# brdav/refign

Measured on AMD Instinct MI355X. Metric: image-pairs/s (align+seg fwd+bwd, 1080x1920), higher is better.
Workload: dtype bf16

## Files before the change

### refign_amd/csrc/attn.hip

```cpp
#include <cstdlib>

#include "common.h"
#include "mfma.h"

namespace rfn {

constexpr int kPackBlock = 4096;
constexpr float kLog2e = 1.4426950408889634f;

__global__ __launch_bounds__(256) void attn_pack_kernel(const uint16_t* __restrict__ src0, const uint16_t* __restrict__ src1,
                                                        long sb, long sr, int heads, int nrows, int nblk,
                                                        unsigned char* __restrict__ rpack0, unsigned char* __restrict__ tpack0,
                                                        unsigned char* __restrict__ rpack1, unsigned char* __restrict__ tpack1) {
  __shared__ unsigned tile[32][33];
  const uint16_t* src = blockIdx.z ? src1 : src0;
  unsigned char* rpack = blockIdx.z ? rpack1 : rpack0;
  unsigned char* tpack = blockIdx.z ? tpack1 : tpack0;
  const int blk = blockIdx.x, bh = blockIdx.y;
  const int b = bh / heads, hd = bh % heads;
  const int t = threadIdx.x, row = t >> 3, dc = t & 7;
  const int grow = blk * 32 + row;
  u32x4 v = {0u, 0u, 0u, 0u};
  if (grow < nrows) v = *(const u32x4*)(src + (long)b * sb + (long)grow * sr + hd * 64 + dc * 8);
  unsigned char* rb = rpack + ((long)bh * nblk + blk) * kPackBlock;
  if (rpack != nullptr) *(u32x4*)(rb + (dc * 32 + row) * 16) = v;
  if (tpack == nullptr) return;
  tile[row][dc * 4 + 0] = v[0];
  tile[row][dc * 4 + 1] = v[1];
  tile[row][dc * 4 + 2] = v[2];
  tile[row][dc * 4 + 3] = v[3];
  __syncthreads();
  const int rq = t >> 5, dp = t & 31;
  unsigned r0 = tile[4 * rq + 0][dp], r1 = tile[4 * rq + 1][dp], r2 = tile[4 * rq + 2][dp], r3 = tile[4 * rq + 3][dp];
  u32x4 o;
  o[0] = (r0 & 0xffffu) | (r1 << 16);
  o[1] = (r2 & 0xffffu) | (r3 << 16);
  o[2] = (r0 >> 16) | (r1 & 0xffff0000u);
  o[3] = (r2 >> 16) | (r3 & 0xffff0000u);
  unsigned char* tb = tpack + ((long)bh * nblk + blk) * kPackBlock;
  *(u32x4*)(tb + (rq * 64 + 2 * dp) * 8) = o;
}

template <int DT>
__device__ __forceinline__ void load_row_frags(const uint16_t* base, long row_stride, int row, int nrows, int g,
                                               typename Elem<DT>::vec8 (&f)[4]) {
  const bool ok = row < nrows;
  const uint16_t* p = base + (long)(ok ? row : 0) * row_stride + 8 * g;
#pragma unroll
  for (int ks = 0; ks < 4; ++ks) {
    u32x4 v = {0u, 0u, 0u, 0u};
    if (ok) v = *(const u32x4*)(p + 16 * ks);
    f[ks] = __builtin_bit_cast(typename Elem<DT>::vec8, v);
  }
}

template <int DT>
__device__ __forceinline__ void store_rows64(const f32x16 (&acc)[2], float mul, uint16_t* rowptr, bool ok, int g) {
#pragma unroll
  for (int db = 0; db < 2; ++db) {
    u32x2 pk[4];
#pragma unroll
    for (int k = 0; k < 4; ++k)
      pk[k] = pack4<DT>(acc[db][4 * k] * mul, acc[db][4 * k + 1] * mul, acc[db][4 * k + 2] * mul, acc[db][4 * k + 3] * mul);
#pragma unroll
    for (int p = 0; p < 2; ++p) {
      auto r0 = __builtin_amdgcn_permlane32_swap(pk[2 * p][0], pk[2 * p + 1][0], false, false);
      auto r1 = __builtin_amdgcn_permlane32_swap(pk[2 * p][1], pk[2 * p + 1][1], false, false);
      if (ok) {
        u32x4 o = {r0[0], r1[0], r0[1], r1[1]};
        *(u32x4*)(rowptr + db * 32 + 16 * p + 8 * g) = o;
      }
    }
  }
}

template <int DT>
__device__ __forceinline__ void to_operands(const float (&p)[16], typename Elem<DT>::vec8 (&b)[2]) {
#pragma unroll
  for (int m = 0; m < 2; ++m)
    b[m] = join8<DT>(pack4<DT>(p[8 * m], p[8 * m + 1], p[8 * m + 2], p[8 * m + 3]),
                     pack4<DT>(p[8 * m + 4], p[8 * m + 5], p[8 * m + 6], p[8 * m + 7]));
}

template <int DT>
__global__ __launch_bounds__(256) void attn_fwd_kernel(const uint16_t* __restrict__ Q, long qsb, long qsr,
                                                       const unsigned char* __restrict__ Kr,
                                                       const unsigned char* __restrict__ Vt, uint16_t* __restrict__ O,
                                                       long osb, long osr, float* __restrict__ lse2, int heads, int Nq,
                                                       int Nkv, int nblk, int nqpad, float scale, int pheads) {
  using E = Elem<DT>;
  using vec8 = typename E::vec8;
  constexpr int STAGE = 4 * kPackBlock;
  __shared__ __attribute__((aligned(16))) unsigned char smem[2 * STAGE];
  const int lane = threadIdx.x & 63, wave = threadIdx.x >> 6, g = lane >> 5, col = lane & 31;
  const int bh = blockIdx.y, b = bh / heads, hd = bh % heads;
  const int q = blockIdx.x * 128 + wave * 32 + col;
  const float c = scale * kLog2e;

  vec8 qf[4];
  load_row_frags<DT>(Q + (long)b * qsb + hd * 64, qsr, q, Nq, g, qf);
#pragma unroll
  for (int kk = 0; kk < 4; ++kk) pin_loaded(qf[kk]);

  const long pidx = (long)(b * pheads + hd) * nblk * kPackBlock;
  const unsigned char* kbase = Kr + pidx;
  const unsigned char* vbase = Vt + pidx;
  const int nst = nblk / 2;
  auto issue = [&](int st, int buf) {
    unsigned char* dst = smem + buf * STAGE;
#pragma unroll
    for (int u = 0; u < 2; ++u) {
      const int piece = wave * 2 + u;
      lds_dma16(kbase + (long)st * 2 * kPackBlock + piece * 1024 + lane * 16, dst + piece * 1024);
      lds_dma16(vbase + (long)st * 2 * kPackBlock + piece * 1024 + lane * 16, dst + 2 * kPackBlock + piece * 1024);
    }
  };

  f32x16 oacc[2];
#pragma unroll
  for (int r = 0; r < 16; ++r) oacc[0][r] = oacc[1][r] = 0.f;
  float mrun = -1e30f, lrun = 0.f;

  issue(0, 0);
  wait_dma_all();
  wg_barrier();
  for (int st = 0; st < nst; ++st) {
    const int buf = st & 1;
    if (st + 1 < nst) issue(st + 1, buf ^ 1);
    const unsigned char* ks = smem + buf * STAGE;
    const unsigned char* vs = ks + 2 * kPackBlock;
    const int key0 = st * 64;
    f32x16 sacc[2];
#pragma unroll
    for (int kb = 0; kb < 2; ++kb)
#pragma unroll
      for (int r = 0; r < 16; ++r) sacc[kb][r] = 0.f;
    {
      vec8 kfr[4];
      auto kfrag = [&](int idx) {
        return *(const vec8*)(ks + (idx >> 2) * kPackBlock + ((2 * (idx & 3) + g) * 32 + col) * 16);
      };
#pragma unroll
      for (int idx = 0; idx < 4; ++idx) kfr[idx] = kfrag(idx);
      __builtin_amdgcn_sched_barrier(0);
#pragma unroll
      for (int idx = 0; idx < 8; ++idx) {
        sacc[idx >> 2] = E::mma(kfr[idx & 3], qf[idx & 3], sacc[idx >> 2]);
        if (idx + 4 < 8) kfr[idx & 3] = kfrag(idx + 4);
        __builtin_amdgcn_sched_barrier(0);
      }
    }
    vec8 vfr[4];
    auto vfrag = [&](int idx) {
      const unsigned char* vq = vs + (idx >> 2) * kPackBlock + ((idx & 1) * 32 + col) * 8;
      const int m = (idx >> 1) & 1;
      return join8<DT>(*(const u32x2*)(vq + (4 * m + g) * 512), *(const u32x2*)(vq + (4 * m + 2 + g) * 512));
    };
#pragma unroll
    for (int idx = 0; idx < 4; ++idx) vfr[idx] = vfrag(idx);
    __builtin_amdgcn_sched_barrier(0);
    float p[2][16];
#pragma unroll
    for (int kb = 0; kb < 2; ++kb)
#pragma unroll
      for (int r = 0; r < 16; ++r) p[kb][r] = sacc[kb][r];
    if (key0 + 64 > Nkv) {
      asm volatile("; padded keys" ::: "memory");
#pragma unroll
      for (int kb = 0; kb < 2; ++kb)
#pragma unroll
        for (int r = 0; r < 16; ++r)
          if (key0 + kb * 32 + (r & 3) + 8 * (r >> 2) + 4 * g >= Nkv) p[kb][r] = -1e30f;
    }
    float mt = p[0][0];
#pragma unroll
    for (int kb = 0; kb < 2; ++kb)
#pragma unroll
      for (int r = 0; r < 16; ++r) mt = fmaxf(mt, p[kb][r]);
    mt = half_max(mt) * c;
    const float mnew = fmaxf(mrun, mt);
    if (__any(mnew > mrun)) {
      const float alpha = __builtin_amdgcn_exp2f(mrun - mnew);
      lrun *= alpha;
#pragma unroll
      for (int r = 0; r < 16; ++r) {
        oacc[0][r] *= alpha;
        oacc[1][r] *= alpha;
      }
      mrun = mnew;
    }
    float ps = 0.f;
#pragma unroll
    for (int kb = 0; kb < 2; ++kb)
#pragma unroll
      for (int r = 0; r < 16; ++r) {
        p[kb][r] = __builtin_amdgcn_exp2f(__builtin_fmaf(p[kb][r], c, -mrun));
        ps += p[kb][r];
      }
    lrun += ps;
    {
      vec8 pb[2][2];
      to_operands<DT>(p[0], pb[0]);
      to_operands<DT>(p[1], pb[1]);
#pragma unroll
      for (int idx = 0; idx < 8; ++idx) {
        const int kb = idx >> 2, m = (idx >> 1) & 1, db = idx & 1;
        oacc[db] = E::mma(vfr[idx & 3], pb[kb][m], oacc[db]);
        if (idx + 4 < 8) vfr[idx & 3] = vfrag(idx + 4);
        __builtin_amdgcn_sched_barrier(0);
      }
    }
    wait_dma_all();
    wg_barrier();
  }
  const float l = half_sum(lrun);
  const bool ok = q < Nq;
  store_rows64<DT>(oacc, 1.f / l, O + (long)b * osb + (long)(ok ? q : 0) * osr + hd * 64, ok, g);
  if (g == 0 && q < nqpad) lse2[(long)bh * nqpad + q] = ok ? mrun + log2f(l) : 0.f;
}


template <int DT>
__global__ __launch_bounds__(256) void attn_bwd_dq_kernel(const uint16_t* __restrict__ Q, long qsb, long qsr,
                                                          const uint16_t* __restrict__ dO, const uint16_t* __restrict__ O,
                                                          long osb, long osr, const unsigned char* __restrict__ Kr,
                                                          const unsigned char* __restrict__ Vr,
                                                          const unsigned char* __restrict__ Kt,
                                                          const float* __restrict__ lse2, float* __restrict__ delta,
                                                          uint16_t* __restrict__ dQ, long dsb, long dsr, int heads, int Nq,
                                                          int Nkv, int nblk, int nqpad, float scale, int pheads) {
  using E = Elem<DT>;
  using vec8 = typename E::vec8;
  constexpr int STAGE = 6 * kPackBlock;
  __shared__ __attribute__((aligned(16))) unsigned char smem[2 * STAGE];
  const int lane = threadIdx.x & 63, wave = threadIdx.x >> 6, g = lane >> 5, col = lane & 31;
  const int bh = blockIdx.y, b = bh / heads, hd = bh % heads;
  const int q = blockIdx.x * 128 + wave * 32 + col;
  const bool ok = q < Nq;
  const float c = scale * kLog2e;

  vec8 qf[4], gf[4];
  load_row_frags<DT>(Q + (long)b * qsb + hd * 64, qsr, q, Nq, g, qf);
  load_row_frags<DT>(dO + (long)b * osb + hd * 64, osr, q, Nq, g, gf);
  float dl = 0.f;
  {
    vec8 of[4];
    load_row_frags<DT>(O + (long)b * osb + hd * 64, osr, q, Nq, g, of);
#pragma unroll
    for (int kk = 0; kk < 4; ++kk)
#pragma unroll
      for (int e = 0; e < 8; ++e) dl += (float)gf[kk][e] * (float)of[kk][e];
    dl = half_sum(dl);
  }
  const float ls = (q < nqpad) ? lse2[(long)bh * nqpad + q] : 0.f;
  if (g == 0 && q < nqpad) delta[(long)bh * nqpad + q] = ok ? dl : 0.f;
#pragma unroll
  for (int kk = 0; kk < 4; ++kk) {
    pin_loaded(qf[kk]);
    pin_loaded(gf[kk]);
  }
  pin_loaded(ls);

  const long pbase = (long)(b * pheads + hd) * nblk * kPackBlock;
  const int nst = nblk / 2;
  auto issue = [&](int st, int buf) {
    unsigned char* dst = smem + buf * STAGE;
#pragma unroll
    for (int u = 0; u < 2; ++u) {
      const int piece = wave * 2 + u;
      const long off = pbase + (long)st * 2 * kPackBlock + piece * 1024 + lane * 16;
      lds_dma16(Kr + off, dst + piece * 1024);
      lds_dma16(Vr + off, dst + 2 * kPackBlock + piece * 1024);
      lds_dma16(Kt + off, dst + 4 * kPackBlock + piece * 1024);
    }
  };

  f32x16 dq[2];
#pragma unroll
  for (int r = 0; r < 16; ++r) dq[0][r] = dq[1][r] = 0.f;

  issue(0, 0);
  wait_dma_all();
  wg_barrier();
  for (int st = 0; st < nst; ++st) {
    const int buf = st & 1;
    if (st + 1 < nst) issue(st + 1, buf ^ 1);
    const unsigned char* base = smem + buf * STAGE;
    const int key0 = st * 64;
    f32x16 sacc[2], dpacc[2];
#pragma unroll
    for (int kb = 0; kb < 2; ++kb)
#pragma unroll
      for (int r = 0; r < 16; ++r) sacc[kb][r] = dpacc[kb][r] = 0.f;
    {
      vec8 fr[4];
      auto frag = [&](int idx) {
        const int kb = idx >> 3, kk = (idx >> 1) & 3;
        return *(const vec8*)(base + ((idx & 1) * 2 + kb) * kPackBlock + ((2 * kk + g) * 32 + col) * 16);
      };
#pragma unroll
      for (int idx = 0; idx < 4; ++idx) fr[idx] = frag(idx);
      __builtin_amdgcn_sched_barrier(0);
#pragma unroll
      for (int idx = 0; idx < 16; ++idx) {
        const int kb = idx >> 3, kk = (idx >> 1) & 3;
        if (idx & 1) dpacc[kb] = E::mma(fr[idx & 3], gf[kk], dpacc[kb]);
        else sacc[kb] = E::mma(fr[idx & 3], qf[kk], sacc[kb]);
        if (idx + 4 < 16) fr[idx & 3] = frag(idx + 4);
        __builtin_amdgcn_sched_barrier(0);
      }
    }
    vec8 ktf[4];
    auto ktfrag = [&](int idx) {
      const unsigned char* kq = base + (4 + (idx >> 2)) * kPackBlock + ((idx & 1) * 32 + col) * 8;
      const int m = (idx >> 1) & 1;
      return join8<DT>(*(const u32x2*)(kq + (4 * m + g) * 512), *(const u32x2*)(kq + (4 * m + 2 + g) * 512));
    };
#pragma unroll
    for (int idx = 0; idx < 4; ++idx) ktf[idx] = ktfrag(idx);
    __builtin_amdgcn_sched_barrier(0);
    float ds[2][16];
#pragma unroll
    for (int kb = 0; kb < 2; ++kb)
#pragma unroll
      for (int r = 0; r < 16; ++r)
        ds[kb][r] = __builtin_amdgcn_exp2f(__builtin_fmaf(sacc[kb][r], c, -ls)) * (dpacc[kb][r] - dl);
    if (key0 + 64 > Nkv) {
      asm volatile("; padded keys" ::: "memory");
#pragma unroll
      for (int kb = 0; kb < 2; ++kb)
#pragma unroll
        for (int r = 0; r < 16; ++r)
          if (key0 + kb * 32 + (r & 3) + 8 * (r >> 2) + 4 * g >= Nkv) ds[kb][r] = 0.f;
    }
    {
      vec8 sb[2][2];
      to_operands<DT>(ds[0], sb[0]);
      to_operands<DT>(ds[1], sb[1]);
#pragma unroll
      for (int idx = 0; idx < 8; ++idx) {
        dq[idx & 1] = E::mma(ktf[idx & 3], sb[idx >> 2][(idx >> 1) & 1], dq[idx & 1]);
        if (idx + 4 < 8) ktf[idx & 3] = ktfrag(idx + 4);
        __builtin_amdgcn_sched_barrier(0);
      }
    }
    wait_dma_all();
    wg_barrier();
  }
  store_rows64<DT>(dq, scale, dQ + (long)b * dsb + (long)(ok ? q : 0) * dsr + hd * 64, ok, g);
}

template <int DT, int NS>
__global__ __launch_bounds__(512) void attn_bwd_dkv_kernel(const uint16_t* __restrict__ K, const uint16_t* __restrict__ V,
                                                           long ksb, long ksr, const unsigned char* __restrict__ Qr,
                                                           const unsigned char* __restrict__ Qt,
                                                           const unsigned char* __restrict__ Gr,
                                                           const unsigned char* __restrict__ Gt,
                                                           const float* __restrict__ lse2, const float* __restrict__ delta,
                                                           float* __restrict__ accT, int heads, int Nq, int Nkv, int nqblk,
                                                           int nqpad, int nkpad, int blocks_per_chunk, float scale) {
  using E = Elem<DT>;
  using vec8 = typename E::vec8;
  constexpr int STATS = 4 * kPackBlock;
  constexpr int STAGE = STATS + 256;
  __shared__ __attribute__((aligned(16))) unsigned char smem[NS * STAGE];
  const int lane = threadIdx.x & 63, wave = threadIdx.x >> 6, g = lane >> 5, col = lane & 31;
  const int bh = blockIdx.z, b = bh / heads, hd = bh % heads;
  const int key = blockIdx.x * 256 + wave * 32 + col;
  const bool wave_live = blockIdx.x * 256 + wave * 32 < Nkv;
  const bool kok = key < Nkv;
  const float c = scale * kLog2e;

  vec8 kf[4], vf[4];
  load_row_frags<DT>(K + (long)b * ksb + hd * 64, ksr, key, Nkv, g, kf);
  load_row_frags<DT>(V + (long)b * ksb + hd * 64, ksr, key, Nkv, g, vf);
#pragma unroll
  for (int kk = 0; kk < 4; ++kk) {
    pin_loaded(kf[kk]);
    pin_loaded(vf[kk]);
  }

  const int qb0 = blockIdx.y * blocks_per_chunk;
  const int nst = min(qb0 + blocks_per_chunk, nqblk) - qb0;
  const long pbase = (long)bh * nqblk * kPackBlock;
  const float* stat_src = (g == 0 ? lse2 : delta) + (long)bh * nqpad + col;
  auto issue = [&](int qb, int buf) {
    unsigned char* dst = smem + buf * STAGE;
    const long off = pbase + (long)qb * kPackBlock + (wave & 3) * 1024 + lane * 16;
    if (wave < 4) {
      lds_dma16(Qr + off, dst + (wave & 3) * 1024);
      lds_dma16(Gr + off, dst + kPackBlock + (wave & 3) * 1024);
    } else {
      lds_dma16(Qt + off, dst + 2 * kPackBlock + (wave & 3) * 1024);
      lds_dma16(Gt + off, dst + 3 * kPackBlock + (wave & 3) * 1024);
    }
    if (wave == 0) lds_dma4(stat_src + qb * 32, dst + STATS);
  };

  f32x16 dk[2], dv[2];
#pragma unroll
  for (int r = 0; r < 16; ++r) dk[0][r] = dk[1][r] = dv[0][r] = dv[1][r] = 0.f;

#pragma unroll
  for (int s = 0; s < NS - 1; ++s)
    if (s < nst) issue(qb0 + s, s);
  for (int i = 0; i < nst; ++i) {
    if (NS == 2 || i + NS - 2 >= nst) wait_dma_all();
    else if (wave == 0) wait_dma_upto<(NS - 2) * 3>();
    else wait_dma_upto<(NS - 2) * 2>();
    wg_barrier();
    if (i + NS - 1 < nst) issue(qb0 + i + NS - 1, (i + NS - 1) % NS);
    if (wave_live) {
      const unsigned char* base = smem + (i % NS) * STAGE;
      f32x4 l4[4], d4[4];
#pragma unroll
      for (int k = 0; k < 4; ++k) {
        l4[k] = *(const f32x4*)(base + STATS + (8 * k + 4 * g) * 4);
        d4[k] = *(const f32x4*)(base + STATS + 128 + (8 * k + 4 * g) * 4);
      }
      f32x16 s, dp;
#pragma unroll
      for (int r = 0; r < 16; ++r) s[r] = dp[r] = 0.f;
      {
        vec8 fr[4];
        auto frag = [&](int idx) {
          return *(const vec8*)(base + (idx & 1) * kPackBlock + ((2 * (idx >> 1) + g) * 32 + col) * 16);
        };
#pragma unroll
        for (int idx = 0; idx < 4; ++idx) fr[idx] = frag(idx);
        __builtin_amdgcn_sched_barrier(0);
#pragma unroll
        for (int idx = 0; idx < 8; ++idx) {
          if (idx & 1) dp = E::mma(fr[idx & 3], vf[idx >> 1], dp);
          else s = E::mma(fr[idx & 3], kf[idx >> 1], s);
          if (idx + 4 < 8) fr[idx & 3] = frag(idx + 4);
          __builtin_amdgcn_sched_barrier(0);
        }
      }
      vec8 tf[4];
      auto tfrag = [&](int idx) {
        const int m = idx >> 2, db = (idx >> 1) & 1;
        const unsigned char* pq = base + (2 + ((idx & 1) ^ 1)) * kPackBlock + (db * 32 + col) * 8;
        return join8<DT>(*(const u32x2*)(pq + (4 * m + g) * 512), *(const u32x2*)(pq + (4 * m + 2 + g) * 512));
      };
#pragma unroll
      for (int idx = 0; idx < 4; ++idx) tf[idx] = tfrag(idx);
      __builtin_amdgcn_sched_barrier(0);
      float p[16], ds[16];
#pragma unroll
      for (int r = 0; r < 16; ++r) {
        float pr = __builtin_amdgcn_exp2f(__builtin_fmaf(s[r], c, -l4[r >> 2][r & 3]));
        if (!kok) pr = 0.f;
        p[r] = pr;
        ds[r] = pr * (dp[r] - d4[r >> 2][r & 3]);
      }
      vec8 pb[2], sb[2];
      to_operands<DT>(p, pb);
      to_operands<DT>(ds, sb);
#pragma unroll
      for (int idx = 0; idx < 8; ++idx) {
        const int m = idx >> 2, db = (idx >> 1) & 1;
        if (idx & 1) dk[db] = E::mma(tf[idx & 3], sb[m], dk[db]);
        else dv[db] = E::mma(tf[idx & 3], pb[m], dv[db]);
        if (idx + 4 < 8) tf[idx & 3] = tfrag(idx + 4);
        __builtin_amdgcn_sched_barrier(0);
      }
    }
  }
  if (kok) {
    float* ak = accT + (long)bh * 2 * 64 * nkpad + key;
    float* av = ak + (long)64 * nkpad;
#pragma unroll
    for (int db = 0; db < 2; ++db)
#pragma unroll
      for (int r = 0; r < 16; ++r) {
        const int d = db * 32 + (r & 3) + 8 * (r >> 2) + 4 * g;
        atomicAdd(ak + (long)d * nkpad, dk[db][r] * scale);
        atomicAdd(av + (long)d * nkpad, dv[db][r]);
      }
  }
}

template <int DT>
__global__ __launch_bounds__(256) void attn_dkv_finish_kernel(const float* __restrict__ accT, uint16_t* __restrict__ dkv,
                                                              int heads, int Nkv, int nkpad, long total) {
  using S = typename Elem<DT>::scalar;
  const long i = (long)blockIdx.x * 256 + threadIdx.x;
  if (i >= total) return;
  const int d = (int)(i & 63);
  long r = i >> 6;
  const int hd = (int)(r % heads);
  r /= heads;
  const int which = (int)(r & 1);
  r >>= 1;
  const int key = (int)(r % Nkv);
  const int b = (int)(r / Nkv);
  const float v = accT[(((long)(b * heads + hd) * 2 + which) * 64 + d) * nkpad + key];
  const S o = (S)v;
  dkv[i] = __builtin_bit_cast(uint16_t, o);
}

}

extern "C" {

using namespace rfn;

#define ATTN_DT_OK(dt) RFN_REQUIRE((dt) == 1 || (dt) == 2, "attention: dtype %d (1 = bf16, 2 = f16)", (dt))

int rfn_attn_pack(const void* src, long batch_stride, long row_stride, int B, int heads, int nrows, int nblk, void* rpack,
                  void* tpack, const void* src2, void* rpack2, void* tpack2, rfn_stream_t stream) {
  RFN_REQUIRE(src && (rpack || tpack), "attn_pack: null pointer");
  RFN_REQUIRE(src2 == nullptr || rpack2 || tpack2, "attn_pack: second tensor without outputs");
  RFN_REQUIRE(B > 0 && heads > 0 && nrows > 0 && nblk * 32 >= nrows, "attn_pack: B=%d heads=%d rows=%d nblk=%d", B, heads,
              nrows, nblk);
  RFN_REQUIRE(row_stride % 8 == 0 && batch_stride % 8 == 0, "attn_pack: strides must be multiples of 8 elements");
  dim3 grid(nblk, B * heads, src2 ? 2 : 1);
  hipLaunchKernelGGL(attn_pack_kernel, grid, dim3(256), 0, (hipStream_t)stream, (const uint16_t*)src,
                     (const uint16_t*)src2, batch_stride, row_stride, heads, nrows, nblk, (unsigned char*)rpack,
                     (unsigned char*)tpack, (unsigned char*)rpack2, (unsigned char*)tpack2);
  return check_launch("attn_pack");
}

int rfn_attn_fwd(const void* Q, long q_batch_stride, long q_row_stride, const void* k_rpack, const void* v_tpack, void* O,
                 long o_batch_stride, long o_row_stride, float* lse2, int B, int heads, int Nq, int Nkv, int nkblk,
                 int nqpad, float scale, int kv_pack_heads, int dtype, rfn_stream_t stream) {
  ATTN_DT_OK(dtype);
  RFN_REQUIRE(Q && k_rpack && v_tpack && O && lse2, "attn_fwd: null pointer");
  RFN_REQUIRE(B > 0 && heads > 0 && Nq > 0 && Nkv > 0 && nkblk % 2 == 0 && nkblk * 32 >= Nkv && nqpad >= Nq,
              "attn_fwd: B=%d heads=%d Nq=%d Nkv=%d nkblk=%d nqpad=%d", B, heads, Nq, Nkv, nkblk, nqpad);
  RFN_REQUIRE(q_row_stride % 8 == 0 && o_row_stride % 8 == 0 && q_batch_stride % 8 == 0 && o_batch_stride % 8 == 0,
              "attn_fwd: strides must be multiples of 8 elements");
  RFN_REQUIRE(kv_pack_heads >= heads, "attn_fwd: kv_pack_heads");
  dim3 grid(cdiv(Nq, 128), B * heads);
  if (dtype == 1)
    hipLaunchKernelGGL(attn_fwd_kernel<1>, grid, dim3(256), 0, (hipStream_t)stream, (const uint16_t*)Q, q_batch_stride,
                       q_row_stride, (const unsigned char*)k_rpack, (const unsigned char*)v_tpack, (uint16_t*)O,
                       o_batch_stride, o_row_stride, lse2, heads, Nq, Nkv, nkblk, nqpad, scale, kv_pack_heads);
  else
    hipLaunchKernelGGL(attn_fwd_kernel<2>, grid, dim3(256), 0, (hipStream_t)stream, (const uint16_t*)Q, q_batch_stride,
                       q_row_stride, (const unsigned char*)k_rpack, (const unsigned char*)v_tpack, (uint16_t*)O,
                       o_batch_stride, o_row_stride, lse2, heads, Nq, Nkv, nkblk, nqpad, scale, kv_pack_heads);
  return check_launch("attn_fwd");
}

int rfn_attn_bwd_dq(const void* Q, long q_batch_stride, long q_row_stride, const void* dO, const void* O,
                    long o_batch_stride, long o_row_stride, const void* k_rpack, const void* v_rpack, const void* k_tpack,
                    const float* lse2, float* delta, void* dQ, long dq_batch_stride, long dq_row_stride, int B, int heads,
                    int Nq, int Nkv, int nkblk, int nqpad, float scale, int kv_pack_heads, int dtype,
                    rfn_stream_t stream) {
  ATTN_DT_OK(dtype);
  RFN_REQUIRE(Q && dO && O && k_rpack && v_rpack && k_tpack && lse2 && delta && dQ, "attn_bwd_dq: null pointer");
  RFN_REQUIRE(B > 0 && heads > 0 && Nq > 0 && Nkv > 0 && nkblk % 2 == 0 && nkblk * 32 >= Nkv && nqpad >= Nq,
              "attn_bwd_dq: B=%d heads=%d Nq=%d Nkv=%d nkblk=%d nqpad=%d", B, heads, Nq, Nkv, nkblk, nqpad);
  dim3 grid(cdiv(Nq, 128), B * heads);
#define RFN_DQ_LAUNCH(D)                                                                                                \
  hipLaunchKernelGGL(attn_bwd_dq_kernel<D>, grid, dim3(256), 0, (hipStream_t)stream, (const uint16_t*)Q, q_batch_stride, \
                     q_row_stride, (const uint16_t*)dO, (const uint16_t*)O, o_batch_stride, o_row_stride,               \
                     (const unsigned char*)k_rpack, (const unsigned char*)v_rpack, (const unsigned char*)k_tpack, lse2,  \
                     delta, (uint16_t*)dQ, dq_batch_stride, dq_row_stride, heads, Nq, Nkv, nkblk, nqpad, scale,          \
                     kv_pack_heads)
  if (dtype == 1) RFN_DQ_LAUNCH(1); else RFN_DQ_LAUNCH(2);
#undef RFN_DQ_LAUNCH
  return check_launch("attn_bwd_dq");
}

int rfn_attn_bwd_dkv(const void* K, const void* V, long kv_batch_stride, long kv_row_stride, const void* q_rpack,
                     const void* q_tpack, const void* do_rpack, const void* do_tpack, const float* lse2,
                     const float* delta, float* accT, void* dKV, int B, int heads, int Nq, int Nkv, int nqblk, int nqpad,
                     int nkpad, int blocks_per_chunk, float scale, int dtype, rfn_stream_t stream) {
  ATTN_DT_OK(dtype);
  RFN_REQUIRE(K && V && q_rpack && q_tpack && do_rpack && do_tpack && lse2 && delta && accT && dKV,
              "attn_bwd_dkv: null pointer");
  RFN_REQUIRE(B > 0 && heads > 0 && Nq > 0 && Nkv > 0 && nqblk * 32 >= Nq && nqpad >= nqblk * 32 && nkpad >= Nkv &&
                  nkpad % 32 == 0 && blocks_per_chunk > 0,
              "attn_bwd_dkv: B=%d heads=%d Nq=%d Nkv=%d nqblk=%d nqpad=%d nkpad=%d chunk=%d", B, heads, Nq, Nkv, nqblk,
              nqpad, nkpad, blocks_per_chunk);
  hipStream_t s = (hipStream_t)stream;
  if (int rc = zero_async(accT, (size_t)B * heads * 2 * 64 * nkpad * sizeof(float), s)) return rc;
  dim3 grid(cdiv(Nkv, 256), cdiv(nqblk, blocks_per_chunk), B * heads);
  static const int ring = 2;
#define RFN_DKV_LAUNCH_(D, R)                                                                                           \
  hipLaunchKernelGGL((attn_bwd_dkv_kernel<D, R>), grid, dim3(512), 0, s, (const uint16_t*)K, (const uint16_t*)V,            \
                     kv_batch_stride, kv_row_stride, (const unsigned char*)q_rpack, (const unsigned char*)q_tpack,      \
                     (const unsigned char*)do_rpack, (const unsigned char*)do_tpack, lse2, delta, accT, heads, Nq, Nkv,  \
                     nqblk, nqpad, nkpad, blocks_per_chunk, scale)
#define RFN_DKV_LAUNCH(D)                                                                                               \
  switch (ring) {                                                                                                       \
    case 4: RFN_DKV_LAUNCH_(D, 4); break;                                                                               \
    default: RFN_DKV_LAUNCH_(D, 2); break;                                                                              \
  }
  if (dtype == 1) { RFN_DKV_LAUNCH(1) } else { RFN_DKV_LAUNCH(2) }
#undef RFN_DKV_LAUNCH
#undef RFN_DKV_LAUNCH_
  int rc = check_launch("attn_bwd_dkv");
  if (rc != RFN_OK) return rc;
  const long total = (long)B * Nkv * 2 * heads * 64;
  if (dtype == 1)
    hipLaunchKernelGGL(attn_dkv_finish_kernel<1>, dim3(cdiv(total, 256)), dim3(256), 0, s, accT, (uint16_t*)dKV, heads,
                       Nkv, nkpad, total);
  else
    hipLaunchKernelGGL(attn_dkv_finish_kernel<2>, dim3(cdiv(total, 256)), dim3(256), 0, s, accT, (uint16_t*)dKV, heads,
                       Nkv, nkpad, total);
  return check_launch("attn_dkv_finish");
}

}
```

### refign_amd/mfma.py

```python
import ctypes
import os

import torch

from . import _lib
from ._tensor import current_stream, on_device, ptr

_DT16 = {torch.bfloat16: 1, torch.float16: 2}
ENABLED = True

LIBRARY_CALLS = {}
_NOTE = True


def note_library(kind, *tensors):
    if not _NOTE or not tensors or not tensors[0].is_cuda:
        return
    key = (kind, str(tensors[0].dtype).replace("torch.", ""), tuple(tuple(t.shape) for t in tensors))
    n = LIBRARY_CALLS.get(key)
    if n is None and len(LIBRARY_CALLS) < 4096:
        if os.environ.get("RFN_LOG_LIBRARY", "0") == "1":
            print(f"[refign_amd] library fallback: {kind} {key[1]} {key[2]}", flush=True)
        LIBRARY_CALLS[key] = 1
    elif n is not None:
        LIBRARY_CALLS[key] = n + 1


def library_summary():
    out = {}
    for (kind, dt, _), n in LIBRARY_CALLS.items():
        e = out.setdefault(f"{kind}/{dt}", {"calls": 0, "shapes": 0})
        e["calls"] += n
        e["shapes"] += 1
    return out


def _row_major(t):
    return t.dim() == 2 and t.stride(1) == 1 and t.stride(0) % 8 == 0 and t.stride(0) >= t.shape[1] \
        and t.data_ptr() % 16 == 0


def gemm_nt(x, w, bias=None, res=None, rowscale=None, rows_per_sample=0, act=0, out=None):
    if not (ENABLED and x.is_cuda and x.dtype in _DT16 and w.dtype == x.dtype and _row_major(x) and _row_major(w)):
        return None
    M, K = x.shape
    N = w.shape[0]
    if w.shape[1] != K or K % 64 != 0 or N % 8 != 0 or M == 0:
        return None
    if bias is not None and not (bias.dtype == x.dtype and bias.is_contiguous() and bias.numel() == N):
        return None
    if out is None:
        out = torch.empty((M, N), dtype=x.dtype, device=x.device)
    if res is not None and not (res.dtype == x.dtype and res.shape == out.shape and res.stride() == out.stride()):
        return None
    if rowscale is not None and (rows_per_sample <= 0 or rowscale.dtype != torch.float32 or not rowscale.is_contiguous()):
        return None
    lib = _lib.load_library()
    with on_device(x.device):
        rc = lib.rfn_gemm_nt(ptr(x), ptr(w), ptr(bias), ptr(res), ptr(rowscale), int(rows_per_sample), int(act),
                             ptr(out), M, N, K, x.stride(0), w.stride(0), out.stride(0), _DT16[x.dtype],
                             current_stream(x.device))
    _lib.check(rc, "gemm_nt")
    return out


def pack_conv_weight(w, dtype, scale=None):
    N, C, KH, KW = w.shape
    Cp = -(-C // 8) * 8
    K = KH * KW * Cp
    Kp = -(-K // 64) * 64
    wf = w.float() if scale is None else w.float() * scale.float().view(-1, 1, 1, 1)
    out = torch.zeros((N, Kp), dtype=dtype, device=w.device)
    t = torch.zeros((N, KH, KW, Cp), dtype=torch.float32, device=w.device)
    t[..., :C] = wf.permute(0, 2, 3, 1)
    out[:, :K] = t.reshape(N, K).to(dtype)
    return out


def conv2d_nhwc(x, wp, bias, KH, KW, stride=1, pad=0, dil=1, act=0, res=None, out=None):
    if not (ENABLED and x.is_cuda and x.dtype in _DT16 and wp.dtype == x.dtype and x.dim() == 4 and x.is_contiguous()
            and x.shape[-1] % 8 == 0 and wp.is_contiguous()):
        return None
    B, H, W, C = x.shape
    N = wp.shape[0]
    if N % 8 != 0 or wp.shape[1] < KH * KW * C or wp.shape[1] % 64 != 0:
        return None
    OH = (H + 2 * pad - dil * (KH - 1) - 1) // stride + 1
    OW = (W + 2 * pad - dil * (KW - 1) - 1) // stride + 1
    if out is None:
        out = torch.empty((B, OH, OW, N), dtype=x.dtype, device=x.device)
    if tuple(out.shape) != (B, OH, OW, N) or out.stride(3) != 1 or out.stride(2) % 8 != 0 or \
            out.stride(1) != OW * out.stride(2) or out.stride(0) != OH * out.stride(1):
        return None
    if res is not None and (res.dtype != x.dtype or res.shape != out.shape or res.stride() != out.stride()):
        return None
    if bias is not None and not (bias.dtype == x.dtype and bias.is_contiguous() and bias.numel() == N):
        return None
    lib = _lib.load_library()
    with on_device(x.device):
        rc = lib.rfn_conv2d_nhwc(ptr(x), ptr(wp), ptr(bias), ptr(res), int(act), ptr(out), B, H, W, C, N, KH, KW, stride,
                                 pad, dil, wp.stride(0), out.stride(2), _DT16[x.dtype], current_stream(x.device))
    _lib.check(rc, "conv2d_nhwc")
    return out


def conv2d_nhwc_dgrad(gy, wt, H, W, C, KH, KW, stride=1, pad=0, dil=1):
    if not (ENABLED and gy.is_cuda and gy.dtype in _DT16 and wt.dtype == gy.dtype and gy.dim() == 4 and gy.is_contiguous()
            and wt.is_contiguous() and stride & (stride - 1) == 0):
        return None
    B, OH, OW, N = gy.shape
    if N % 8 or C % 8 or wt.shape[0] != C or wt.shape[1] < KH * KW * N or wt.shape[1] % 64:
        return None
    if (OH, OW) != ((H + 2 * pad - dil * (KH - 1) - 1) // stride + 1, (W + 2 * pad - dil * (KW - 1) - 1) // stride + 1):
        return None
    dx = torch.empty((B, H, W, C), dtype=gy.dtype, device=gy.device)
    with on_device(gy.device):
        rc = _lib.load_library().rfn_conv2d_nhwc_dgrad(ptr(gy), ptr(wt), ptr(dx), B, H, W, C, N, KH, KW, stride, pad, dil,
                                                       wt.stride(0), C, _DT16[gy.dtype], current_stream(gy.device))
    _lib.check(rc, "conv2d_nhwc_dgrad")
    return dx


def conv2d_nhwc_wgrad(gy, x, KH, KW, Kpad, stride=1, pad=0, dil=1, bias_out=None):
    if not (ENABLED and gy.is_cuda and gy.dtype in _DT16 and x.dtype == gy.dtype and gy.dim() == 4 and x.dim() == 4
            and gy.is_contiguous() and x.is_contiguous()):
        return None
    B, OH, OW, N = gy.shape
    _, H, W, C = x.shape
    if N % 64 or C % 2 or Kpad % 64 or Kpad < KH * KW * C or Kpad >= 65536 or x.shape[0] != B:
        return None
    if (OH, OW) != ((H + 2 * pad - dil * (KH - 1) - 1) // stride + 1, (W + 2 * pad - dil * (KW - 1) - 1) // stride + 1):
        return None
    T = B * OH * OW
    tile = 128 if (N % 128 == 0 and Kpad % 128 == 0) else 64
    rows = slab_rows(T, (N // tile) * (Kpad // tile))
    S = -(-T // rows)
    part = torch.empty((S, N, Kpad), dtype=torch.float32, device=gy.device)
    with on_device(gy.device):
        rc = _lib.load_library().rfn_conv2d_nhwc_wgrad(ptr(gy), ptr(x), ptr(part), ptr(bias_out), B, H, W, C, N, KH, KW, stride,
                                                       pad, dil, N, Kpad, rows, 0, _DT16[gy.dtype], current_stream(gy.device))
    _lib.check(rc, "conv2d_nhwc_wgrad")
    return part


_TN_WGS = 1024


_TN_ATOMICS = 2500000
_TN_MIN_WGS = 512


def slab_rows(T, tiles, nk=0):
    want = max(1, min(64, _TN_WGS // max(tiles, 1)))
    if nk > 0:
        want = min(want, max(4, _TN_ATOMICS // nk, -(-_TN_MIN_WGS // max(tiles, 1))))
    rows = -(-T // want)
    rows = max(256, -(-rows // 32) * 32)
    return rows


def gemm_tn(g, x, rows_per_slab=None, out=None, bias_out=None, rowscale=None, rows_per_sample=0):
    if not (ENABLED and g.is_cuda and g.dtype in _DT16 and x.dtype == g.dtype and g.dim() == 2 and x.dim() == 2
            and g.stride(1) == 1 and x.stride(1) == 1 and g.stride(0) % 2 == 0 and x.stride(0) % 2 == 0
            and g.data_ptr() % 4 == 0 and x.data_ptr() % 4 == 0):
        return None
    T, N = g.shape
    K = x.shape[1]
    if x.shape[0] != T or N % 64 != 0 or K % 64 != 0 or T == 0:
        return None
    if rowscale is not None and not (rowscale.dtype == torch.float32 and rowscale.is_contiguous() and rows_per_sample > 0
                                     and rowscale.numel() * rows_per_sample >= T):
        return None
    if rows_per_slab is None:
        tile = 128 if (N % 128 == 0 and K % 128 == 0) else 64
        rows_per_slab = slab_rows(T, (N // tile) * (K // tile), N * K)
    S = -(-T // rows_per_slab)
    if out is not None:
        if not (out.dtype == torch.float32 and out.is_contiguous() and out.numel() == N * K and
                (bias_out is None or (bias_out.dtype == torch.float32 and bias_out.is_contiguous()
                                      and bias_out.numel() == N))):
            return None
        part = out
    else:
        part = torch.empty((S, N, K), dtype=torch.float32, device=g.device)
    lib = _lib.load_library()
    with on_device(g.device):
        rc = lib.rfn_gemm_tn(ptr(g), ptr(x), ptr(part), T, N, K, g.stride(0), x.stride(0), int(rows_per_slab),
                             0 if out is None else 1, ptr(bias_out) if out is not None else None, ptr(rowscale),
                             int(rows_per_sample), _DT16[g.dtype], current_stream(g.device))
    _lib.check(rc, "gemm_tn")
    return part


GROUP_WGRADS = True
_TN_GROUP_MAX = 8
_WGRAD_QUEUE = None


def _tn_domain(g, x, rowscale, rows_per_sample):
    if not (ENABLED and g.is_cuda and g.dtype in _DT16 and x.dtype == g.dtype and g.dim() == 2 and x.dim() == 2
            and g.stride(1) == 1 and x.stride(1) == 1 and g.stride(0) % 2 == 0 and x.stride(0) % 2 == 0
            and g.data_ptr() % 4 == 0 and x.data_ptr() % 4 == 0):
        return False
    T, N = g.shape
    K = x.shape[1]
    if x.shape[0] != T or N % 64 != 0 or K % 64 != 0 or T == 0:
        return False
    if rowscale is not None and not (rowscale.dtype == torch.float32 and rowscale.is_contiguous() and rows_per_sample > 0
                                     and rowscale.numel() * rows_per_sample >= T):
        return False
    return True


def defer_gemm_tn(g, x, out, bias_out=None, rowscale=None, rows_per_sample=0):
    q = _WGRAD_QUEUE
    if q is None or not _tn_domain(g, x, rowscale, rows_per_sample):
        return False
    T, N = g.shape
    K = x.shape[1]
    if not (out.dtype == torch.float32 and out.is_contiguous() and out.numel() == N * K and
            (bias_out is None or (bias_out.dtype == torch.float32 and bias_out.is_contiguous() and bias_out.numel() == N))):
        return False
    if g.stride(0) % 8 or x.stride(0) % 8 or g.data_ptr() % 16 or x.data_ptr() % 16:
        return False
    rows = slab_rows(T, (N // 64) * (K // 64), N * K)
    if rowscale is not None and (rows + rows_per_sample - 1) // rows_per_sample + 1 > 64:
        return False
    q.append((g, x, out, bias_out, rowscale, int(rows_per_sample), int(rows)))
    return True


def flush_wgrads():
    q = _WGRAD_QUEUE
    if not q:
        return
    items, q[:] = list(q), []
    classes = {}
    for it in items:
        classes.setdefault((it[4] is not None, it[0].dtype, it[0].device), []).append(it)
    lib = _lib.load_library()
    vp, lg, it_ = ctypes.c_void_p, ctypes.c_long, ctypes.c_int
    for (seg, dt, dev), lst in classes.items():
        for a in range(0, len(lst), _TN_GROUP_MAX):
            grp = lst[a:a + _TN_GROUP_MAX]
            n = len(grp)
            arr = lambda ty, vals: (ty * n)(*vals)
            G = arr(vp, [t[0].data_ptr() for t in grp])
            X = arr(vp, [t[1].data_ptr() for t in grp])
            P = arr(vp, [t[2].data_ptr() for t in grp])
            Bv = arr(vp, [None if t[3] is None else t[3].data_ptr() for t in grp])
            R = arr(vp, [None if t[4] is None else t[4].data_ptr() for t in grp])
            T = arr(lg, [t[0].shape[0] for t in grp])
            N = arr(lg, [t[0].shape[1] for t in grp])
            K = arr(lg, [t[1].shape[1] for t in grp])
            ldg = arr(lg, [t[0].stride(0) for t in grp])
            ldx = arr(lg, [t[1].stride(0) for t in grp])
            rps = arr(it_, [t[6] for t in grp])
            rsa = arr(it_, [t[5] for t in grp])
            cast = lambda a_: ctypes.cast(a_, vp)
            with on_device(dev):
                rc = lib.rfn_gemm_tn_grouped(n, cast(G), cast(X), cast(P), cast(Bv), cast(R), cast(T), cast(N), cast(K),
                                             cast(ldg), cast(ldx), cast(rps), cast(rsa), _DT16[dt], current_stream(dev))
            _lib.check(rc, "gemm_tn_grouped")


class deferred_wgrads:

    def __enter__(self):
        global _WGRAD_QUEUE
        self._outer = _WGRAD_QUEUE
        if GROUP_WGRADS and ENABLED and self._outer is None:
            _WGRAD_QUEUE = []
        return self

    def __exit__(self, *exc):
        global _WGRAD_QUEUE
        if self._outer is None and _WGRAD_QUEUE is not None:
            try:
                if exc[0] is None:
                    flush_wgrads()
            finally:
                _WGRAD_QUEUE = None
        return False


class _WgradMark(torch.autograd.Function):

    @staticmethod
    def forward(ctx, x):
        return x.view_as(x)

    @staticmethod
    def backward(ctx, g):
        flush_wgrads()
        return g


def wgrad_mark(x):
    return _WgradMark.apply(x) if (GROUP_WGRADS and torch.is_grad_enabled() and x.requires_grad) else x


_PACK_BLOCK = 4096


def _pack(src, batch_stride, row_stride, B, heads, nrows, nblk, want_r=True, want_t=True, src2=None):
    dev = src.device
    nbytes = B * heads * nblk * _PACK_BLOCK
    new = lambda want: torch.empty(nbytes, dtype=torch.uint8, device=dev) if want else None
    r, t = new(want_r), new(want_t)
    r2, t2 = (new(want_r), new(want_t)) if src2 is not None else (None, None)
    lib = _lib.load_library()
    with on_device(dev):
        rc = lib.rfn_attn_pack(ptr(src), batch_stride, row_stride, B, heads, nrows, nblk, ptr(r), ptr(t), ptr(src2),
                               ptr(r2), ptr(t2), current_stream(dev))
    _lib.check(rc, "attn_pack")
    return (r, t), (r2, t2)


def _attn_ok(q, kv, heads):
    if not (ENABLED and q.is_cuda and q.dtype in _DT16 and kv.dtype == q.dtype and q.dim() == 3 and kv.dim() == 3):
        return False
    B, N, C = q.shape
    return (C == heads * 64 and kv.shape[0] == B and kv.shape[2] == 2 * C and q.is_contiguous() and kv.is_contiguous()
            and q.data_ptr() % 16 == 0 and kv.data_ptr() % 16 == 0)


def _dims(q, kv):
    B, N, C = q.shape
    Nkv = kv.shape[1]
    nkblk = -(-Nkv // 32)
    nkblk += nkblk & 1
    nqblk = -(-N // 32)
    return B, N, C, Nkv, nkblk, nqblk, nqblk * 32


def _fwd(q, kv, heads, scale, need_bwd):
    B, N, C, Nkv, nkblk, nqblk, nqpad = _dims(q, kv)
    dev = q.device
    (kvr, kvt), _ = _pack(kv, kv.stride(0), kv.stride(1), B, 2 * heads, Nkv, nkblk)
    voff = heads * nkblk * _PACK_BLOCK
    o = torch.empty_like(q)
    lse2 = torch.empty((B * heads, nqpad), dtype=torch.float32, device=dev)
    lib = _lib.load_library()
    with on_device(dev):
        rc = lib.rfn_attn_fwd(ptr(q), q.stride(0), q.stride(1), kvr.data_ptr(), kvt.data_ptr() + voff, ptr(o),
                              o.stride(0), o.stride(1), ptr(lse2), B, heads, N, Nkv, nkblk, nqpad, float(scale),
                              2 * heads, _DT16[q.dtype], current_stream(dev))
    _lib.check(rc, "attn_fwd")
    return o, lse2, (kvr, kvt)


def _chunk_blocks(nqblk, Nkv, BH):
    kblocks = -(-Nkv // 256)
    chunks = max(1, 128 // max(1, kblocks * BH))
    return max(4, -(-nqblk // chunks))


class _AttnFn(torch.autograd.Function):
    @staticmethod
    def forward(ctx, q, kv, heads, scale):
        need = q.requires_grad or kv.requires_grad
        o, lse2, packs = _fwd(q, kv, heads, scale, need)
        if need:
            ctx.save_for_backward(q, kv, o, lse2, *packs)
            ctx.heads, ctx.scale = heads, scale
        return o

    @staticmethod
    def backward(ctx, do):
        q, kv, o, lse2, kvr, kvt = ctx.saved_tensors
        heads, scale = ctx.heads, ctx.scale
        B, N, C, Nkv, nkblk, nqblk, nqpad = _dims(q, kv)
        dev = q.device
        if do.dtype != q.dtype:
            do = do.to(q.dtype)
        if not do.is_contiguous():
            do = do.contiguous()
        dt = _DT16[q.dtype]
        lib = _lib.load_library()
        dq = torch.empty_like(q)
        delta = torch.empty_like(lse2)
        voff = heads * nkblk * _PACK_BLOCK
        with on_device(dev):
            rc = lib.rfn_attn_bwd_dq(ptr(q), q.stride(0), q.stride(1), ptr(do), ptr(o), o.stride(0), o.stride(1),
                                     kvr.data_ptr(), kvr.data_ptr() + voff, kvt.data_ptr(), ptr(lse2), ptr(delta),
                                     ptr(dq), dq.stride(0), dq.stride(1), B, heads, N, Nkv, nkblk, nqpad, float(scale),
                                     2 * heads, dt, current_stream(dev))
        _lib.check(rc, "attn_bwd_dq")
        (qr, qt), (gr, gt) = _pack(q, q.stride(0), q.stride(1), B, heads, N, nqblk, src2=do)
        nkpad = -(-Nkv // 32) * 32
        accT = torch.empty(B * heads * 2 * 64 * nkpad, dtype=torch.float32, device=dev)
        dkv = torch.empty_like(kv)
        k_view, v_view = kv[:, :, :C], kv[:, :, C:]
        with on_device(dev):
            rc = lib.rfn_attn_bwd_dkv(ptr(k_view), ptr(v_view), kv.stride(0), kv.stride(1), ptr(qr), ptr(qt), ptr(gr),
                                      ptr(gt), ptr(lse2), ptr(delta), ptr(accT), ptr(dkv), B, heads, N, Nkv, nqblk,
                                      nqpad, nkpad, _chunk_blocks(nqblk, Nkv, B * heads), float(scale), dt,
                                      current_stream(dev))
        _lib.check(rc, "attn_bwd_dkv")
        return dq, dkv, None, None


def attention(q, kv, heads, scale):
    if not _attn_ok(q, kv, heads):
        return None
    return _AttnFn.apply(q, kv, heads, scale)
```

Before: 16.68.

## Software-pipeline attention forward: overlap next-tile QK with current softmax and PV

Restructures the flash-attention forward loop so the score MFMAs for the next key tile are interleaved with the exponentials of the current tile, and the row-max of the next tile is interleaved with the PV MFMAs. K and V are split into separately double-buffered LDS regions, and padding masking is specialised to the tail steps only. The running-max rescale now fires only when the max grows by more than a threshold, and max3 instructions shorten the reduction. In the no-grad path the host packs only the K row-pack and the V transposed pack instead of both for all heads. This adds register pressure and relies on the lazy rescale staying numerically safe in bf16.

```diff
diff --git a/refign_amd/csrc/attn.hip b/refign_amd/csrc/attn.hip
--- a/refign_amd/csrc/attn.hip
+++ b/refign_amd/csrc/attn.hip
@@ -1,4 +1,5 @@
 #include <cstdlib>
+#include <type_traits>
 
 #include "common.h"
 #include "mfma.h"
@@ -82,6 +83,14 @@
                      pack4<DT>(p[8 * m + 4], p[8 * m + 5], p[8 * m + 6], p[8 * m + 7]));
 }
 
+constexpr float kRescaleThr = 8.f;
+
+__device__ __forceinline__ float max3f(float a, float b, float c) {
+  float r;
+  asm("v_max3_f32 %0, %1, %2, %3" : "=v"(r) : "v"(a), "v"(b), "v"(c));
+  return r;
+}
+
 template <int DT>
 __global__ __launch_bounds__(256) void attn_fwd_kernel(const uint16_t* __restrict__ Q, long qsb, long qsr,
                                                        const unsigned char* __restrict__ Kr,
@@ -90,8 +99,8 @@
                                                        int Nkv, int nblk, int nqpad, float scale, int pheads) {
   using E = Elem<DT>;
   using vec8 = typename E::vec8;
-  constexpr int STAGE = 4 * kPackBlock;
-  __shared__ __attribute__((aligned(16))) unsigned char smem[2 * STAGE];
+  constexpr int HALF = 2 * kPackBlock;
+  __shared__ __attribute__((aligned(16))) unsigned char smem[4 * HALF];
   const int lane = threadIdx.x & 63, wave = threadIdx.x >> 6, g = lane >> 5, col = lane & 31;
   const int bh = blockIdx.y, b = bh / heads, hd = bh % heads;
   const int q = blockIdx.x * 128 + wave * 32 + col;
@@ -106,80 +115,142 @@
   const unsigned char* kbase = Kr + pidx;
   const unsigned char* vbase = Vt + pidx;
   const int nst = nblk / 2;
-  auto issue = [&](int st, int buf) {
-    unsigned char* dst = smem + buf * STAGE;
+  auto issue_k = [&](int st) {
 #pragma unroll
     for (int u = 0; u < 2; ++u) {
       const int piece = wave * 2 + u;
-      lds_dma16(kbase + (long)st * 2 * kPackBlock + piece * 1024 + lane * 16, dst + piece * 1024);
-      lds_dma16(vbase + (long)st * 2 * kPackBlock + piece * 1024 + lane * 16, dst + 2 * kPackBlock + piece * 1024);
-    }
+      lds_dma16(kbase + (long)st * HALF + piece * 1024 + lane * 16, smem + (st & 1) * HALF + piece * 1024);
+    }
+  };
+  auto issue_v = [&](int st) {
+#pragma unroll
+    for (int u = 0; u < 2; ++u) {
+      const int piece = wave * 2 + u;
+      lds_dma16(vbase + (long)st * HALF + piece * 1024 + lane * 16, smem + (2 + (st & 1)) * HALF + piece * 1024);
+    }
+  };
+  auto kfrag = [&](int st, int idx) {
+    return *(const vec8*)(smem + (st & 1) * HALF + (idx >> 2) * kPackBlock + ((2 * (idx & 3) + g) * 32 + col) * 16);
+  };
+  auto vfrag = [&](int st, int idx) {
+    const unsigned char* vq = smem + (2 + (st & 1)) * HALF + (idx >> 2) * kPackBlock + ((idx & 1) * 32 + col) * 8;
+    const int m = (idx >> 1) & 1;
+    return join8<DT>(*(const u32x2*)(vq + (4 * m + g) * 512), *(const u32x2*)(vq + (4 * m + 2 + g) * 512));
+  };
+  auto pad_mask = [&](f32x16 (&s)[2], int st) {
+    const int lim = Nkv - st * 64 - 4 * g;
+#pragma unroll
+    for (int kb = 0; kb < 2; ++kb)
+#pragma unroll
+      for (int r = 0; r < 16; ++r)
+        if (kb * 32 + (r & 3) + 8 * (r >> 2) >= lim) s[kb][r] = -1e30f;
+  };
+  auto rowmax = [&](const f32x16 (&s)[2]) {
+    float m0 = max3f(s[0][0], s[0][1], s[0][2]), m1 = max3f(s[1][0], s[1][1], s[1][2]);
+#pragma unroll
+    for (int r = 3; r < 15; r += 2) {
+      m0 = max3f(m0, s[0][r], s[0][r + 1]);
+      m1 = max3f(m1, s[1][r], s[1][r + 1]);
+    }
+    return half_max(max3f(m0, m1, max3f(s[0][15], s[1][15], s[1][15]))) * c;
   };
 
   f32x16 oacc[2];
 #pragma unroll
   for (int r = 0; r < 16; ++r) oacc[0][r] = oacc[1][r] = 0.f;
-  float mrun = -1e30f, lrun = 0.f;
-
-  issue(0, 0);
+  float lrun = 0.f;
+
+  auto scores = [&](f32x16 (&s)[2], int st) {
+    vec8 kfr[4];
+#pragma unroll
+    for (int idx = 0; idx < 4; ++idx) kfr[idx] = kfrag(st, idx);
+#pragma unroll
+    for (int idx = 0; idx < 8; ++idx) {
+      s[idx >> 2] = E::mma(kfr[idx & 3], qf[idx & 3], (idx & 3) ? s[idx >> 2] : f32x16{});
+      if (idx + 4 < 8) kfr[idx & 3] = kfrag(st, idx + 4);
+    }
+  };
+  auto probs = [&](const f32x16 (&s)[2], float m, vec8 (&pb)[2][2]) {
+    float ps = 0.f;
+#pragma unroll
+    for (int kb = 0; kb < 2; ++kb) {
+      float p[16];
+#pragma unroll
+      for (int r = 0; r < 16; ++r) {
+        p[r] = __builtin_amdgcn_exp2f(__builtin_fmaf(s[kb][r], c, -m));
+        ps += p[r];
+      }
+      to_operands<DT>(p, pb[kb]);
+    }
+    return ps;
+  };
+
+  f32x16 sa[2], sb[2];
+  issue_k(0);
+  issue_v(0);
+  if (nst > 1) issue_k(1);
   wait_dma_all();
   wg_barrier();
-  for (int st = 0; st < nst; ++st) {
-    const int buf = st & 1;
-    if (st + 1 < nst) issue(st + 1, buf ^ 1);
-    const unsigned char* ks = smem + buf * STAGE;
-    const unsigned char* vs = ks + 2 * kPackBlock;
-    const int key0 = st * 64;
-    f32x16 sacc[2];
-#pragma unroll
-    for (int kb = 0; kb < 2; ++kb)
-#pragma unroll
-      for (int r = 0; r < 16; ++r) sacc[kb][r] = 0.f;
+  scores(sa, 0);
+  if (nst == 1) pad_mask(sa, 0);
+  float mrun = rowmax(sa);
+
+  auto step = [&](f32x16 (&sc)[2], f32x16 (&sn)[2], int st, auto pad) {
+    wait_dma_all();
+    wg_barrier();
+    if (st + 2 < nst) issue_k(st + 2);
+    issue_v(st + 1);
+    u32x2 pk[8];
+    float ps = 0.f;
     {
       vec8 kfr[4];
-      auto kfrag = [&](int idx) {
-        return *(const vec8*)(ks + (idx >> 2) * kPackBlock + ((2 * (idx & 3) + g) * 32 + col) * 16);
-      };
-#pragma unroll
-      for (int idx = 0; idx < 4; ++idx) kfr[idx] = kfrag(idx);
+#pragma unroll
+      for (int idx = 0; idx < 4; ++idx) kfr[idx] = kfrag(st + 1, idx);
       __builtin_amdgcn_sched_barrier(0);
 #pragma unroll
-      for (int idx = 0; idx < 8; ++idx) {
-        sacc[idx >> 2] = E::mma(kfr[idx & 3], qf[idx & 3], sacc[idx >> 2]);
-        if (idx + 4 < 8) kfr[idx & 3] = kfrag(idx + 4);
+      for (int i = 0; i < 8; ++i) {
+        sn[i >> 2] = E::mma(kfr[i & 3], qf[i & 3], (i & 3) ? sn[i >> 2] : f32x16{});
+        if (i + 4 < 8) kfr[i & 3] = kfrag(st + 1, i + 4);
+        float p4[4];
+#pragma unroll
+        for (int e = 0; e < 4; ++e) {
+          p4[e] = __builtin_amdgcn_exp2f(__builtin_fmaf(sc[i >> 2][4 * (i & 3) + e], c, -mrun));
+          ps += p4[e];
+        }
+        pk[i] = pack4<DT>(p4[0], p4[1], p4[2], p4[3]);
         __builtin_amdgcn_sched_barrier(0);
       }
     }
-    vec8 vfr[4];
-    auto vfrag = [&](int idx) {
-      const unsigned char* vq = vs + (idx >> 2) * kPackBlock + ((idx & 1) * 32 + col) * 8;
-      const int m = (idx >> 1) & 1;
-      return join8<DT>(*(const u32x2*)(vq + (4 * m + g) * 512), *(const u32x2*)(vq + (4 * m + 2 + g) * 512));
-    };
-#pragma unroll
-    for (int idx = 0; idx < 4; ++idx) vfr[idx] = vfrag(idx);
-    __builtin_amdgcn_sched_barrier(0);
-    float p[2][16];
-#pragma unroll
-    for (int kb = 0; kb < 2; ++kb)
-#pragma unroll
-      for (int r = 0; r < 16; ++r) p[kb][r] = sacc[kb][r];
-    if (key0 + 64 > Nkv) {
-      asm volatile("; padded keys" ::: "memory");
-#pragma unroll
-      for (int kb = 0; kb < 2; ++kb)
-#pragma unroll
-        for (int r = 0; r < 16; ++r)
-          if (key0 + kb * 32 + (r & 3) + 8 * (r >> 2) + 4 * g >= Nkv) p[kb][r] = -1e30f;
-    }
-    float mt = p[0][0];
-#pragma unroll
-    for (int kb = 0; kb < 2; ++kb)
-#pragma unroll
-      for (int r = 0; r < 16; ++r) mt = fmaxf(mt, p[kb][r]);
-    mt = half_max(mt) * c;
-    const float mnew = fmaxf(mrun, mt);
-    if (__any(mnew > mrun)) {
+    lrun += ps;
+    if constexpr (decltype(pad)::value) pad_mask(sn, st + 1);
+    float mt;
+    {
+      vec8 vfr[4];
+#pragma unroll
+      for (int idx = 0; idx < 4; ++idx) vfr[idx] = vfrag(st, idx);
+      __builtin_amdgcn_sched_barrier(0);
+      float m0 = 0.f, m1 = 0.f;
+#pragma unroll
+      for (int i = 0; i < 8; ++i) {
+        const int kb = i >> 2, m = (i >> 1) & 1, db = i & 1;
+        oacc[db] = E::mma(vfr[i & 3], join8<DT>(pk[4 * kb + 2 * m], pk[4 * kb + 2 * m + 1]), oacc[db]);
+        if (i + 4 < 8) vfr[i & 3] = vfrag(st, i + 4);
+        if (i == 0) {
+          m0 = max3f(sn[0][0], sn[0][1], sn[0][2]);
+          m1 = max3f(sn[1][0], sn[1][1], sn[1][2]);
+        } else if (i < 7) {
+          m0 = max3f(m0, sn[0][2 * i + 1], sn[0][2 * i + 2]);
+          m1 = max3f(m1, sn[1][2 * i + 1], sn[1][2 * i + 2]);
+        } else {
+          m0 = max3f(m0, sn[0][15], sn[1][15]);
+          m1 = max3f(m0, m1, m1);
+        }
+        __builtin_amdgcn_sched_barrier(0);
+      }
+      mt = half_max(m1) * c;
+    }
+    if (__any(mt - mrun > kRescaleThr)) {
+      const float mnew = fmaxf(mrun, mt);
       const float alpha = __builtin_amdgcn_exp2f(mrun - mnew);
       lrun *= alpha;
 #pragma unroll
@@ -189,29 +260,41 @@
       }
       mrun = mnew;
     }
-    float ps = 0.f;
-#pragma unroll
-    for (int kb = 0; kb < 2; ++kb)
-#pragma unroll
-      for (int r = 0; r < 16; ++r) {
-        p[kb][r] = __builtin_amdgcn_exp2f(__builtin_fmaf(p[kb][r], c, -mrun));
-        ps += p[kb][r];
-      }
-    lrun += ps;
-    {
-      vec8 pb[2][2];
-      to_operands<DT>(p[0], pb[0]);
-      to_operands<DT>(p[1], pb[1]);
-#pragma unroll
-      for (int idx = 0; idx < 8; ++idx) {
-        const int kb = idx >> 2, m = (idx >> 1) & 1, db = idx & 1;
-        oacc[db] = E::mma(vfr[idx & 3], pb[kb][m], oacc[db]);
-        if (idx + 4 < 8) vfr[idx & 3] = vfrag(idx + 4);
-        __builtin_amdgcn_sched_barrier(0);
-      }
-    }
-    wait_dma_all();
-    wg_barrier();
+  };
+  auto last = [&](const f32x16 (&sc)[2], int st) {
+    if (st > 0) {
+      wait_dma_all();
+      wg_barrier();
+    }
+    vec8 pb[2][2];
+    lrun += probs(sc, mrun, pb);
+    vec8 vfr[4];
+#pragma unroll
+    for (int idx = 0; idx < 4; ++idx) vfr[idx] = vfrag(st, idx);
+#pragma unroll
+    for (int idx = 0; idx < 8; ++idx) {
+      const int kb = idx >> 2, m = (idx >> 1) & 1, db = idx & 1;
+      oacc[db] = E::mma(vfr[idx & 3], pb[kb][m], oacc[db]);
+      if (idx + 4 < 8) vfr[idx & 3] = vfrag(st, idx + 4);
+    }
+  };
+
+  using plain = std::false_type;
+  using padded = std::true_type;
+  int st = 0;
+  for (; st + 3 < nst; st += 2) {
+    step(sa, sb, st, plain{});
+    step(sb, sa, st + 1, plain{});
+  }
+  if (nst - st == 3) {
+    step(sa, sb, st, plain{});
+    step(sb, sa, st + 1, padded{});
+    last(sa, st + 2);
+  } else if (nst - st == 2) {
+    step(sa, sb, st, padded{});
+    last(sb, st + 1);
+  } else {
+    last(sa, st);
   }
   const float l = half_sum(lrun);
   const bool ok = q < Nq;
diff --git a/refign_amd/mfma.py b/refign_amd/mfma.py
--- a/refign_amd/mfma.py
+++ b/refign_amd/mfma.py
@@ -303,12 +303,13 @@
 _PACK_BLOCK = 4096
 
 
-def _pack(src, batch_stride, row_stride, B, heads, nrows, nblk, want_r=True, want_t=True, src2=None):
+def _pack(src, batch_stride, row_stride, B, heads, nrows, nblk, want_r=True, want_t=True, src2=None, want2=None):
     dev = src.device
     nbytes = B * heads * nblk * _PACK_BLOCK
     new = lambda want: torch.empty(nbytes, dtype=torch.uint8, device=dev) if want else None
     r, t = new(want_r), new(want_t)
-    r2, t2 = (new(want_r), new(want_t)) if src2 is not None else (None, None)
+    want_r2, want_t2 = want2 if want2 is not None else (want_r, want_t)
+    r2, t2 = (new(want_r2), new(want_t2)) if src2 is not None else (None, None)
     lib = _lib.load_library()
     with on_device(dev):
         rc = lib.rfn_attn_pack(ptr(src), batch_stride, row_stride, B, heads, nrows, nblk, ptr(r), ptr(t), ptr(src2),
@@ -337,17 +338,23 @@
 def _fwd(q, kv, heads, scale, need_bwd):
     B, N, C, Nkv, nkblk, nqblk, nqpad = _dims(q, kv)
     dev = q.device
-    (kvr, kvt), _ = _pack(kv, kv.stride(0), kv.stride(1), B, 2 * heads, Nkv, nkblk)
-    voff = heads * nkblk * _PACK_BLOCK
+    if need_bwd:
+        (kvr, kvt), _ = _pack(kv, kv.stride(0), kv.stride(1), B, 2 * heads, Nkv, nkblk)
+        kr, vt, pheads = kvr.data_ptr(), kvt.data_ptr() + heads * nkblk * _PACK_BLOCK, 2 * heads
+        packs = (kvr, kvt)
+    else:
+        (kr_t, _), (_, vt_t) = _pack(kv, kv.stride(0), kv.stride(1), B, heads, Nkv, nkblk, want_t=False,
+                                     src2=kv[:, :, C:], want2=(False, True))
+        kr, vt, pheads = kr_t.data_ptr(), vt_t.data_ptr(), heads
+        packs = (kr_t, vt_t)
     o = torch.empty_like(q)
     lse2 = torch.empty((B * heads, nqpad), dtype=torch.float32, device=dev)
     lib = _lib.load_library()
     with on_device(dev):
-        rc = lib.rfn_attn_fwd(ptr(q), q.stride(0), q.stride(1), kvr.data_ptr(), kvt.data_ptr() + voff, ptr(o),
-                              o.stride(0), o.stride(1), ptr(lse2), B, heads, N, Nkv, nkblk, nqpad, float(scale),
-                              2 * heads, _DT16[q.dtype], current_stream(dev))
+        rc = lib.rfn_attn_fwd(ptr(q), q.stride(0), q.stride(1), kr, vt, ptr(o), o.stride(0), o.stride(1), ptr(lse2), B,
+                              heads, N, Nkv, nkblk, nqpad, float(scale), pheads, _DT16[q.dtype], current_stream(dev))
     _lib.check(rc, "attn_fwd")
-    return o, lse2, (kvr, kvt)
+    return o, lse2, packs
 
 
 def _chunk_blocks(nqblk, Nkv, BH):
```

Result: no change. 16.72, median of 6 (+0.2%).
